# ajcm474/gapless-lossy-codec

Hardware: AMD Instinct MI355X
Metric: Msamples/s encoded (48 kHz stereo batch) at 1/2/4/8 GPUs; % HBM roofline (higher is better)
Workload: dtype f32; 1 GPU; BASELINE configs[1]: batch-encode 4096 frames x 1024 samples, 48 kHz stereo synthetic PCM (16-tone chord per channel) per GPU; frames_per_gpu=4096, channels=2, spinup_steps=500

## Files before the change

gapless-lossy-codec_amd/csrc/glc_api.hip:

```cpp
#include <hip/hip_runtime.h>

#include <algorithm>
#include <functional>
#include <cstdio>
#include <memory>
#include <mutex>
#include <new>
#include <string>
#include <cstdlib>
#include <vector>

#include "../../include/glc_debug.h"
#include "glc_args.hpp"
#include "glc_common.h"
#include "glc_kernels.h"
#include "glc_resources.hpp"
#include "glc_rounds.hpp"
#include "glc_stages.hpp"

namespace glc {

static std::mutex g_err_mu;
static std::string g_err;

// ... 48 lines not shown
  DevBuf rtb_stats;
  HostBuf rtb_stage;
  TableImage rtb_image;
  struct RtbClipInfo {
    uint64_t n_frames, stat_off;
    uint32_t stat_slots;
  };
  std::vector<RtbClipInfo> rtb_info;
  uint32_t rtb_info_ch = 0;
  DevBuf cd_status;
  uint64_t cd_status_n = 0;
  DevBuf sc_ws;
  DevBuf sc_stage;
  uint64_t sc_round = 0;
  HostBuf batch_stage;
  std::string err;
  glc::DecodeRows dec_rows{};
  uint64_t dec_uid = 0;
  uint32_t dec_delay = 0;
  uint64_t dec_orig_len = 0, dec_n_pairs = 0, dec_n_raw = 0;
  int d1_variant = 0;
  ScreenPolicy policy;
  HostBuf screen_stat;
  DevBuf edge_failed;
  DevBuf bound_tables;
  HostBuf probe_out;
  uint32_t dec_ch = 0;
  uint64_t dec_frames = 0, dec_next = 0;
  bool stream_open = false;
  int stream_elem = 0;
  DevBuf stream_out;
  int stream_buf = 0;
  uint64_t stream_frames = 0;
  bool stream_last = false;
  Stream own_stream;
  Stream stream;
  Stream copy_stream;
  Stream stream_b;
  Stream down_stream;
  Stream edge_stream;
  Stream probe_stream;
  Event ev_begin, ev_end;
  Event ev_fork, ev_join;
  std::vector<Event> ev_round;
  Event ev_dec[2];
  Event rtb_ev;
  Worker enc_up, enc_launch;
// ... 277 lines not shown
    const glc::SampleWindow need = glc::frame_sample_window(frame_begin, frame_end, plan.per_channel);
    if (need.hi > need.lo && (t0 > need.lo || t0 + t_count < need.hi))
      return fail(ctx, GLC_EINVAL, f + ": PCM shard does not cover the frame range (halo missing)");
  }
  return GLC_OK;
}

static hipError_t launch_quantize_decide(glc_ctx *ctx, const float *coef, const glc::PcmView &view,
                                         uint64_t frame_begin, uint64_t n_frames, uint8_t *records, hipStream_t st) {
  bool decided = false;
  hipError_t e = glc::launch_quantize(ctx->dev, coef, static_cast<uint32_t>(n_frames * view.ch), view.ch, view,
                                      frame_begin, records, st, &decided);
  if (e == hipSuccess && !decided)
    e = glc::launch_decide_raw(ctx->dev, view, frame_begin, static_cast<uint32_t>(n_frames), records, st);
  return e;
}

static hipError_t ensure_screen_shared(glc_ctx *ctx) {
  if (!ctx->screen_stat.p) {
    const hipError_t e = ctx->screen_stat.reserve(2 * 8 * sizeof(uint32_t));
    if (e != hipSuccess) return e;
    std::memset(ctx->screen_stat.p, 0, 2 * 8 * sizeof(uint32_t));
  }
  if (!ctx->edge_failed.p) {
    hipError_t e = ctx->edge_failed.reserve(2 * sizeof(uint64_t));
    if (e == hipSuccess) e = hipMemset(ctx->edge_failed.p, 0, 2 * sizeof(uint64_t));
    if (e == hipSuccess) e = hipStreamSynchronize(nullptr);
    if (e != hipSuccess) return e;
  }
  for (EncodeSlot &s : ctx->slot) {
    s.stat = static_cast<uint32_t *>(ctx->screen_stat.p) + 8 * s.index;
    s.failed_total = static_cast<unsigned long long *>(ctx->edge_failed.p) + s.index;
  }
  return hipSuccess;
}

static hipError_t reserve_slot(glc_ctx *ctx, EncodeSlot &slot, uint32_t ch, uint64_t frames, uint64_t chunk) {
  const uint64_t rows = std::min<uint64_t>(chunk, frames) * ch;
  hipError_t e = slot.coef.reserve(std::max<size_t>(rows, 1) * glc::kHop * sizeof(float));
  if (e == hipSuccess && ctx->policy.workspace_bytes(ch, frames, chunk)) e = ensure_screen_shared(ctx);
  if (e == hipSuccess) e = slot.reserve_screen(ctx->policy, ch, frames, chunk);
  return e;
}

static bool screen_takes(glc_ctx *ctx, uint32_t M, uint32_t ch) {
  ScreenPolicy &pol = ctx->policy;
  if (!pol.may(M, ch)) return false;
  bool pending = false;
  for (EncodeSlot &s : ctx->slot) {
    const volatile uint32_t *hs = s.stat;
    const uint32_t seq = hs[2], failed = hs[0], rows = hs[1];
    pol.observe(s.judged, seq, failed, rows);
    pending = pending || seq != s.seq;
  }
  return pol.admit(pending);
// ... 16 lines not shown
  if (alternate) {
    GLC_HIP(ctx, ctx->stream_b.ensure());
    GLC_HIP(ctx, ctx->ev_fork.ensure());
    GLC_HIP(ctx, ctx->ev_join.ensure());
    GLC_HIP(ctx, reserve_slot(ctx, ctx->slot[1], ch, frame_end - frame_begin, chunk));
    GLC_HIP(ctx, hipEventRecord(ctx->ev_fork, stream));
    GLC_HIP(ctx, hipStreamWaitEvent(ctx->stream_b, ctx->ev_fork, 0));
  }
  const glc_plan plan = glc::plan_encode(view.n_samples, static_cast<uint16_t>(ch));
  const glc::EdgeFrames ef = glc::edge_frames(plan.per_channel, plan.n_frames);
  uint64_t c_idx = 0;
  for (uint64_t f = frame_begin; f < frame_end; f += chunk, ++c_idx) {
    const uint64_t nf = std::min<uint64_t>(chunk, frame_end - f);
    const uint32_t M = static_cast<uint32_t>(nf * ch);
    const bool odd = alternate && (c_idx & 1);
    hipStream_t st = odd ? ctx->stream_b : stream;
    uint8_t *rp = recs + (f - frame_begin) * rec;
    EncodeSlot &slot = odd ? ctx->slot[1] : *r.slot;
    float *coef = d_coeffs ? d_coeffs + (f - frame_begin) * ch * glc::kHop : static_cast<float *>(slot.coef.p);
    if (!d_coeffs && screen_takes(ctx, M, ch)) {
      if (slot.screen_ws.cap < glc::encode_screen_bytes(M, pol.shape))
        return fail(ctx, GLC_EINVAL, "glc_encode_range_device: the screen's workspace was not reserved for this launch");
      bool decided = false;
      glc::ScreenLaunch sl{slot.screen_ws.p, slot.stat, 0, rp, st, pol.latency_repair(), pol.matrix_bound(M, ch), nullptr};
      if (slot.index == 0) pol.tap_rows = M, pol.tap_planes = sl.matrix_bound ? glc::MatrixBound::kGroups : pol.shape.n_planes;
      glc::EdgeLaunch edge{ef.a, ef.b, nullptr, nullptr, nullptr, nullptr, false, nullptr};
      const uint32_t n_edge = glc::edge_rows(ef.a, ef.b, f, M, ch).n;
      if ((flags & kEncodeEdge) && pol.edge_kind != 1 && n_edge >= 1 && n_edge <= glc::kEdgeRowsMax) {
        GLC_HIP(ctx, ctx->edge_stream.ensure());
        for (Event &ev : slot.ev_edge) GLC_HIP(ctx, ev.ensure());
        GLC_HIP(ctx, slot.edge_coef.reserve(static_cast<size_t>(glc::kEdgeRowsMax) * glc::kHop * sizeof(float)));
        edge.side = ctx->edge_stream;
        edge.ev_fork = slot.ev_edge[0], edge.ev_edge = slot.ev_edge[1];
        edge.coef = static_cast<float *>(slot.edge_coef.p);
        edge.capped = pol.edge_capped();
        edge.failed_total = slot.failed_total;
        ++pol.edge_launches;
        pol.edge_rows += n_edge;
        sl.edge = &edge;
      }
      sl.seq = ++slot.seq;
      GLC_HIP(ctx, glc::launch_encode_screened(ctx->dev, pol.shape, view, f, M, coef, sl, &decided));
      ++pol.repair_launches[sl.latency_repair ? 1 : 0];
      if (!decided) GLC_HIP(ctx, glc::launch_decide_raw(ctx->dev, view, f, static_cast<uint32_t>(nf), rp, st));
      pol.rows_screened += M;
      continue;
    }
    GLC_HIP(ctx, glc::launch_mdct_forward(ctx->dev, view, f, M, coef, st, pol.k1_variant, (flags & kEncodeBeside) != 0));
    GLC_HIP(ctx, launch_quantize_decide(ctx, coef, view, f, nf, rp, st));
  }
  if (alternate) {
    GLC_HIP(ctx, hipEventRecord(ctx->ev_join, ctx->stream_b));
    GLC_HIP(ctx, hipStreamWaitEvent(stream, ctx->ev_join, 0));
  }
  return GLC_OK;
}

int glc_encode_range_device(glc_ctx *ctx, const float *d_pcm, uint64_t t0, uint64_t t_count,
                            uint64_t n_samples, uint16_t channels, uint64_t frame_begin,
                            uint64_t frame_end, void *d_records, float *d_coeffs) {
  if (!ctx) return GLC_EINVAL;
  const EncodeRange r{{d_pcm, t0, t_count, n_samples, channels}, frame_begin, frame_end, d_records, d_coeffs, &ctx->slot[0]};
  return encode_range_on(ctx, ctx->stream, r, kEncodeAlternate | kEncodeEdge);
}

// ... 3276 lines not shown
  if (e == hipSuccess) e = hipMemcpy(d, p + 2048 + 4096, 4096, hipMemcpyDeviceToHost);
  GLC_HIP(ctx, e);
  return GLC_OK;
}

int glc_debug_encode_repair_stats(glc_ctx *ctx, uint64_t *launches_tiles, uint64_t *launches_latency) {
  if (!ctx || !launches_tiles || !launches_latency) return fail(ctx, GLC_EINVAL, "glc_debug_encode_repair_stats: null argument");
  *launches_tiles = ctx->policy.repair_launches[0];
  *launches_latency = ctx->policy.repair_launches[1];
  return GLC_OK;
}

int glc_debug_encode_screen_stats(glc_ctx *ctx, uint64_t *rows_screened, uint64_t *rows_repaired) {
  if (!ctx || !rows_screened || !rows_repaired) return fail(ctx, GLC_EINVAL, "glc_debug_encode_screen_stats: null argument");
  DeviceGuard guard(ctx->device);
  GLC_HIP(ctx, hipStreamSynchronize(ctx->stream));
  if (ctx->stream_b) GLC_HIP(ctx, hipStreamSynchronize(ctx->stream_b));
  *rows_screened = ctx->policy.rows_screened;
  *rows_repaired = 0;
  if (ctx->screen_stat.p) {
    const volatile uint64_t *hs = static_cast<const volatile uint64_t *>(ctx->screen_stat.p);
    *rows_repaired = hs[2] + hs[4 + 2];
  }
  if (ctx->edge_failed.p) {
    uint64_t e[2] = {0, 0};
    GLC_HIP(ctx, hipMemcpyAsync(e, ctx->edge_failed.p, sizeof e, hipMemcpyDeviceToHost, ctx->stream));
    GLC_HIP(ctx, hipStreamSynchronize(ctx->stream));
    *rows_repaired += e[0] + e[1];
  }
  return GLC_OK;
}

int glc_debug_encode_screen_layout(uint32_t ne, uint32_t rows, uint32_t *hybrid_pairs, uint32_t *planes,
                                   uint64_t *workspace_bytes) {
  if (!hybrid_pairs || !planes || !workspace_bytes) return GLC_EINVAL;
  const uint32_t edge = 64u * ne;
  glc::ScreenShape sh{};
  if (ne > 16 || !glc::encode_screen_shape(&edge, 1, &sh)) return GLC_EINVAL;
  *hybrid_pairs = sh.hp;
  *planes = sh.n_planes;
  *workspace_bytes = glc::encode_screen_bytes(rows, sh);
  return GLC_OK;
}

int glc_debug_clock_probe_begin(glc_ctx *ctx, uint32_t window_us) {
  if (!ctx || window_us == 0) return fail(ctx, GLC_EINVAL, "glc_debug_clock_probe_begin: bad argument");
  DeviceGuard guard(ctx->device);
  GLC_HIP(ctx, ctx->probe_stream.ensure());
  GLC_HIP(ctx, ctx->probe_out.reserve(64));
  std::memset(ctx->probe_out.p, 0, 16);
  GLC_HIP(ctx, glc::launch_clock_probe(static_cast<uint64_t>(window_us) * 100ull, static_cast<uint64_t *>(ctx->probe_out.p),
                                       ctx->probe_stream));
// ... 45 lines not shown
```

gapless-lossy-codec_amd/csrc/glc_kernels.h:

```cpp
#pragma once
#include <hip/hip_runtime.h>

#include <cstdint>

#include "glc_common.h"

namespace glc {

struct DeviceTables {
  const float *cos_t;
  const float *cos;
  const float *window;
  const float *indiv;
  const float *band_pf;
  const float *band_len;
  const uint16_t *band_of;
  const uint32_t *edges;
  uint32_t n_bands;
  float norm, cf, noise_floor;
  const uint16_t *cos_bf;
};

struct MatrixBound {
  static constexpr int kNe = 6;
// ... 22 lines not shown
};

hipError_t launch_mdct_forward(const DeviceTables &t, const PcmView &pcm, uint64_t frame_begin,
                               uint32_t M, float *coef, hipStream_t s, int variant = 0, bool beside = false);
hipError_t launch_quantize(const DeviceTables &t, const float *coef, uint32_t M, uint32_t ch, const PcmView &pcm,
                           uint64_t frame_begin, uint8_t *records, hipStream_t s, bool *decided);
struct ScreenShape {
  uint32_t l0, c0, ne;
  uint32_t hp;
  uint32_t n_planes;
};
bool encode_screen_shape(const uint32_t *edges, uint32_t n_bands, ScreenShape *sh);
bool mdct_forward_is_st16(uint32_t M, uint32_t ch, int variant);
bool mdct_forward_has_segment_loader(uint32_t ch);
uint64_t encode_screen_bytes(uint32_t M, const ScreenShape &sh);
struct EdgeLaunch {
  uint64_t a, b;
  hipStream_t side;
  hipEvent_t ev_fork, ev_edge;
  float *coef;
  bool capped;
  unsigned long long *failed_total;
};
struct ScreenLaunch {
  void *workspace;
  uint32_t *host_stat;
  uint32_t seq;
  uint8_t *records;
  hipStream_t s;
  bool latency_repair, matrix_bound;
  const EdgeLaunch *edge;
};
hipError_t launch_encode_screened(const DeviceTables &t, const ScreenShape &sh, const PcmView &pcm, uint64_t frame_begin,
                                  uint32_t M, float *coef, const ScreenLaunch &launch, bool *decided);

struct EdgeFrames {
  uint64_t a, b;
};
GLC_HD inline EdgeFrames edge_frames(uint64_t per_channel, uint64_t n_frames) {
  const uint64_t tail = kFrame - kHop / 2;
  uint64_t a = n_frames < 1 ? n_frames : 1;
  uint64_t b = per_channel >= tail ? (per_channel - tail) / kHop + 1 : 0;
  if (b > n_frames) b = n_frames;
  if (b < a) b = a;
  return {a, b};
}
struct EdgeRows {
  unsigned n_pre, suf0, n;
};
// ... 196 lines not shown
```

gapless-lossy-codec_amd/csrc/glc_kernels.hip:

```cpp
#include <algorithm>
#include <type_traits>

#include "glc_common.h"
#include "glc_kernels.h"
#include "glc_mdct_fwd.hpp"

#pragma clang fp contract(off)

namespace glc {

namespace {

template <int FALLBACK = 0, typename F>
auto by_channels(uint32_t ch, F &&f) {
  switch (ch) {
    case 1: return f(std::integral_constant<int, 1>{});
    case 2: return f(std::integral_constant<int, 2>{});
    case 4: return f(std::integral_constant<int, 4>{});
    case 8: return f(std::integral_constant<int, 8>{});
    default: return f(std::integral_constant<int, FALLBACK>{});
  }
}

constexpr int kHopI = 1024;
// ... 12 lines not shown
  return v.p[rel * v.ch + c];
}

__device__ __forceinline__ short sat_i16(float x) {
  if (x != x) return 0;
  x = fminf(fmaxf(x, -32768.0f), 32767.0f);
  return static_cast<short>(static_cast<int>(x));
}


constexpr int kQRows = 4;

constexpr float kScreenCErr = 2.45e-4f, kScreenSlack = 1.001f, kScreenTiny = 1e-33f;

struct ScreenArgs {
  const float *hf;
  unsigned *row_flag;
  unsigned *wave_fail;
  unsigned *host_stat;
  unsigned long long stride;
  unsigned c0, l0, n_planes, seq;
  unsigned long long edge_a, edge_b;
  unsigned long long *edge_total;
};

template <bool FUSED, int MODE>
__device__ __forceinline__ void quantize_body(const DeviceTables &tb, const float *__restrict__ coef, unsigned M,
                                              unsigned ch, unsigned long long rec_bytes, unsigned long long hdr_bytes,
                                              const PcmView &pcm, long long frame_begin,
                                              unsigned char *__restrict__ records, const ScreenArgs &sa) {
  __shared__ __attribute__((aligned(16))) float ssq[4][kQRows][kHopI];
  __shared__ float sbase[4][kQRows][64];
  const int w = threadIdx.x >> 6, lane = threadIdx.x & 63;
  unsigned blk = blockIdx.x;
  EdgeRows er{0u, M, 0u};
  if constexpr (MODE != 0) er = edge_rows(sa.edge_a, sa.edge_b, static_cast<unsigned long long>(frame_begin), M, ch);
  if constexpr (MODE == 3) {
    const unsigned g_pre = (er.n_pre + 15u) / 16u, g_suf = er.suf0 / 16u > g_pre ? er.suf0 / 16u : g_pre;
    if (blk >= g_pre) blk = g_suf + (blk - g_pre);
  }
  const unsigned m0 = (blk * 4 + w) * kQRows;
  unsigned on = 0;
  auto edge_row = [&](unsigned m) -> bool { return m < er.n_pre || m >= er.suf0; };
  if constexpr (MODE == 3) {
#pragma unroll
    for (int r = 0; r < kQRows; ++r)
      if (m0 + r < M && edge_row(m0 + r)) on |= 1u << r;
  }
  if constexpr (MODE == 2) {
    if (blk == 0 && w == 0) {
      const unsigned n_w = (M + 15) / 16 * 4;
      unsigned cnt = 0, ecnt = 0;
      unsigned long long etot = 0;
      if (er.n) etot = *sa.edge_total;
      for (unsigned i = lane; i < n_w; i += 64) cnt += sa.wave_fail[i];
      for (unsigned i = lane; i < er.n; i += 64) ecnt += sa.row_flag[i < er.n_pre ? i : er.suf0 + (i - er.n_pre)] == 2u;
#pragma unroll
      for (int off = 32; off > 0; off >>= 1) cnt += __shfl_xor(cnt, off), ecnt += __shfl_xor(ecnt, off);
      if (lane == 0) {
        volatile unsigned *hs = sa.host_stat;
        volatile unsigned long long *tot = reinterpret_cast<volatile unsigned long long *>(sa.host_stat + 4);
        *tot = *tot + cnt;
        if (er.n) *sa.edge_total = etot + ecnt;
        hs[0] = cnt;
        hs[1] = M;
        hs[2] = sa.seq;
      }
    }
    const unsigned fr = blk * 16 + lane;
    const bool flagged = lane < 16 && fr < M && sa.row_flag[fr] == 1u;
    const unsigned blk_on = static_cast<unsigned>(__ballot(flagged));
    if (blk_on == 0u) return;
    on = (blk_on >> (4 * w)) & 0xFu;
  }
  auto row_on = [&](int r) -> bool {
    if constexpr (MODE == 0) return m0 + r < M;
    else return (on >> r) & 1u;
  };

  float4 indiv4[4];
  unsigned short bo[4][4];
#pragma unroll
  for (int j = 0; j < 4; ++j) {
    const int k0 = (lane + 64 * j) * 4;
    indiv4[j] = *reinterpret_cast<const float4 *>(tb.indiv + k0);
    const ushort4 b4 = *reinterpret_cast<const ushort4 *>(tb.band_of + k0);
    bo[j][0] = b4.x; bo[j][1] = b4.y; bo[j][2] = b4.z; bo[j][3] = b4.w;
  }

  float4 c4[kQRows][4];
  float scale[kQRows];
// ... 56 lines not shown
      const bool pass = __ballot(hit) == 0ull && bound <= nfl && bound < __builtin_inff();
      if (!pass) fail |= 1u << r;
    }
    unsigned valid = 0;
#pragma unroll
    for (int r = 0; r < kQRows; ++r)
      if (m0 + r < M) valid |= 1u << r;
    fail &= valid;
    if (FUSED) {
      unsigned ff = 0;
#pragma unroll
      for (int r = 0; r < kQRows; ++r)
#pragma unroll
        for (int q = 0; q < kQRows; ++q)
          if (static_cast<unsigned>(q) / ch == static_cast<unsigned>(r) / ch && ((fail >> q) & 1u)) ff |= 1u << r;
      fail = ff & valid;
    }
    unsigned edge = 0;
#pragma unroll
    for (int r = 0; r < kQRows; ++r)
      if (((valid >> r) & 1u) && edge_row(m0 + r)) edge |= 1u << r;
    on = valid & ~fail & ~edge;
    if (lane < kQRows && m0 + lane < M) sa.row_flag[m0 + lane] = ((fail >> lane) & 1u) << ((edge >> lane) & 1u);
    if (lane == 0) sa.wave_fail[blk * 4 + w] = __builtin_popcount(fail & ~edge);
  }
  __syncthreads();

  {
    const int r = lane >> 4;
    if (row_on(r)) {
      const float *sq = ssq[w][r];
      for (unsigned b = lane & 15; b < tb.n_bands; b += 16) {
        if constexpr (MODE == 1) {
          if (b == tb.n_bands - 1) {
            sbase[w][r][b] = 0.0f;
            continue;
          }
        }
        const unsigned lo = tb.edges[b], hi = tb.edges[b + 1];
        float ss = 0.0f;
        unsigned i = lo;
        for (; i < hi && (i & 3u); ++i) ss = add_rn(ss, sq[i]);
#define GLC_ADD4(V) ss = add_rn(ss, V.x); ss = add_rn(ss, V.y); ss = add_rn(ss, V.z); ss = add_rn(ss, V.w)
        if (i + 16 <= hi) {
          const float4 *q4 = reinterpret_cast<const float4 *>(sq);
          float4 a0 = q4[i >> 2], a1 = q4[(i >> 2) + 1], a2 = q4[(i >> 2) + 2], a3 = q4[(i >> 2) + 3];
          while (i + 32 <= hi) {
            const float4 b0 = q4[(i >> 2) + 4], b1 = q4[(i >> 2) + 5], b2 = q4[(i >> 2) + 6], b3 = q4[(i >> 2) + 7];
            GLC_ADD4(a0); GLC_ADD4(a1); GLC_ADD4(a2); GLC_ADD4(a3);
// ... 1768 lines not shown
}

hipError_t launch_debug_mfma_bf16(const uint16_t *a, const uint16_t *b, const float *c, float *d, hipStream_t s) {
  hipLaunchKernelGGL(k_debug_mfma_bf16, dim3(1), dim3(64), 0, s, a, b, c, d);
  return hipGetLastError();
}

bool encode_matrix_bound_built(const DeviceTables &t, const ScreenShape &sh, uint32_t ch) {
  return t.cos_bf && sh.ne == static_cast<uint32_t>(MatrixBound::kNe) && (ch == 1 || ch == 2 || ch == 4 || ch == 8);
}

namespace {
inline uint64_t screen_stride(uint32_t M) { return (static_cast<uint64_t>(M) + 255ull) / 256ull * 256ull; }
}

uint64_t encode_screen_bytes(uint32_t M, const ScreenShape &sh) {
  return ((sh.n_planes + 1ull) * screen_stride(M) + screen_stride(M) + screen_stride(M) / 4) * 4ull;
}

hipError_t launch_encode_screened(const DeviceTables &t, const ScreenShape &sh, const PcmView &pcm, uint64_t frame_begin,
                                  uint32_t M, float *coef, const ScreenLaunch &launch, bool *decided) {
  void *const workspace = launch.workspace;
  uint32_t *const host_stat = launch.host_stat;
  const uint32_t seq = launch.seq;
  uint8_t *const records = launch.records;
  const hipStream_t s = launch.s;
  const bool latency_repair = launch.latency_repair, matrix_bound = launch.matrix_bound;
  const EdgeLaunch *const edge = launch.edge;
  *decided = pcm.ch == 1 || pcm.ch == 2 || pcm.ch == 4;
  if (M == 0) return hipSuccess;
  const unsigned long long edge_a = edge ? edge->a : 0ull, edge_b = edge ? edge->b : kNoEdge;
  const EdgeRows er = edge_rows(edge_a, edge_b, frame_begin, M, pcm.ch);
  if (edge && (er.n == 0 || er.n > kEdgeRowsMax || !edge->side || edge->side == s || !edge->coef || !edge->failed_total))
    return hipErrorInvalidValue;
  const uint64_t stride = screen_stride(M);
  float *hf = static_cast<float *>(workspace);
  unsigned *row_flag = reinterpret_cast<unsigned *>(hf + (sh.n_planes + 1ull) * stride);
  unsigned *wave_fail = row_flag + stride;
  static_assert(MatrixBound::kGroups <= 8, "the matrix form's planes fit in those of any FMA form (8 at the least)");
  if (matrix_bound && !encode_matrix_bound_built(t, sh, pcm.ch)) return hipErrorInvalidValue;
  const unsigned n_planes = matrix_bound ? static_cast<unsigned>(MatrixBound::kGroups) : sh.n_planes;
  hipError_t e;
  if (edge && (e = hipEventRecord(edge->ev_fork, s)) != hipSuccess) return e;
  if (matrix_bound)
    e = by_channels<8>(pcm.ch, [&](auto CH) {
      return k1::launch_mx_st<decltype(CH)::value>(t, pcm, frame_begin, M, coef, hf, stride, s);
    });
  else
    e = by_channels(pcm.ch, [&](auto CH) {
      return k1::launch_mix_st<decltype(CH)::value>(t, pcm, frame_begin, M, coef, sh.ne, sh.hp, hf, stride, s);
    });
  if (e != hipSuccess) return e;
  const ScreenArgs sa{hf, row_flag, wave_fail, host_stat, stride, sh.c0, sh.l0, n_planes, seq, edge_a, edge_b,
                      edge ? edge->failed_total : nullptr};
  const unsigned long long hdr = record_header_bytes(pcm.ch), rec = record_bytes(pcm.ch);
  const dim3 grid((M + 4 * kQRows - 1) / (4 * kQRows));
  const long long fb = static_cast<long long>(frame_begin);
  bool forked = false;
  auto leave = [&](hipError_t err) -> hipError_t {
    if (!forked) return err;
    hipError_t j = hipEventRecord(edge->ev_edge, edge->side);
    if (j == hipSuccess) j = hipStreamWaitEvent(s, edge->ev_edge, 0);
    return err != hipSuccess ? err : j;
  };
  if (edge) {
    if ((e = hipStreamWaitEvent(edge->side, edge->ev_fork, 0)) != hipSuccess) return e;
    forked = true;
    e = edge->capped ? k1::launch_edge_rows<GLC_SMALL_ROWS_R, true>(t, pcm, frame_begin, M, edge->coef, er, 0u, edge->side)
                     : k1::launch_edge_rows<GLC_SMALL_ROWS_R, false>(t, pcm, frame_begin, M, edge->coef, er, 0u, edge->side);
    if (e != hipSuccess) return leave(e);
    const unsigned g_pre = (er.n_pre + 15u) / 16u, g_suf = std::max(er.suf0 / 16u, g_pre), g_end = (M + 15u) / 16u;
    const dim3 egrid(g_pre + (er.suf0 < M && g_suf < g_end ? g_end - g_suf : 0u));
    if (*decided)
      hipLaunchKernelGGL((k_quantize_screen<true, 3>), egrid, dim3(256), 0, edge->side, t, edge->coef, M, pcm.ch, rec, hdr, pcm, fb, records, sa);
    else
      hipLaunchKernelGGL((k_quantize_screen<false, 3>), egrid, dim3(256), 0, edge->side, t, edge->coef, M, pcm.ch, rec, hdr, pcm, fb, records, sa);
    if ((e = hipGetLastError()) != hipSuccess) return leave(e);
  }
  if (*decided)
    hipLaunchKernelGGL((k_quantize_screen<true, 1>), grid, dim3(256), 0, s, t, coef, M, pcm.ch, rec, hdr, pcm, fb, records, sa);
  else
    hipLaunchKernelGGL((k_quantize_screen<false, 1>), grid, dim3(256), 0, s, t, coef, M, pcm.ch, rec, hdr, pcm, fb, records, sa);
  if ((e = hipGetLastError()) != hipSuccess) return leave(e);
  e = latency_repair ? k1::launch_small_rows<GLC_SMALL_ROWS_R>(t, pcm, frame_begin, M, coef, row_flag, wave_fail, sh.c0, s)
                     : k1::launch_small_cols<2>(t, pcm, frame_begin, M, coef, row_flag, sh.c0, s);
  if (e != hipSuccess) return leave(e);
  if (*decided)
    hipLaunchKernelGGL((k_quantize_screen<true, 2>), grid, dim3(256), 0, s, t, coef, M, pcm.ch, rec, hdr, pcm, fb, records, sa);
  else
    hipLaunchKernelGGL((k_quantize_screen<false, 2>), grid, dim3(256), 0, s, t, coef, M, pcm.ch, rec, hdr, pcm, fb, records, sa);
  return leave(hipGetLastError());
}

hipError_t launch_quantize(const DeviceTables &t, const float *coef, uint32_t M, uint32_t ch, const PcmView &pcm,
                           uint64_t frame_begin, uint8_t *records, hipStream_t s, bool *decided) {
  *decided = ch == 1 || ch == 2 || ch == 4;
  if (M == 0) return hipSuccess;
  const unsigned long long hdr = record_header_bytes(ch), rec = record_bytes(ch);
  const dim3 grid((M + 4 * kQRows - 1) / (4 * kQRows));
  if (*decided)
    hipLaunchKernelGGL(k_quantize<true>, grid, dim3(256), 0, s, t, coef, M, ch, rec, hdr, pcm,
                       static_cast<long long>(frame_begin), records);
  else
    hipLaunchKernelGGL(k_quantize<false>, grid, dim3(256), 0, s, t, coef, M, ch, rec, hdr, pcm,
                       static_cast<long long>(frame_begin), records);
  return hipGetLastError();
}
// ... 520 lines not shown
```

gapless-lossy-codec_amd/csrc/glc_mdct_fwd.hpp:

```cpp
#pragma once
#include <hip/hip_runtime.h>

#include <type_traits>

#include "glc_kernels.h"

namespace glc {
namespace k1 {

constexpr int kHopI = 1024;
constexpr int kFrameI = 2048;

__device__ __forceinline__ float mul_rn(float a, float b) { return __fmul_rn(a, b); }
__device__ __forceinline__ float add_rn(float a, float b) { return __fadd_rn(a, b); }

typedef float f32x2 __attribute__((ext_vector_type(2)));
typedef float f32x4 __attribute__((ext_vector_type(4)));

template <typename Row, typename Ch>
__device__ __forceinline__ long long pcm_frame_first(const PcmView &pcm, long long frame_begin, Row row, Ch ch) {
  const long long f = frame_begin + row / ch;
  return (f * kHopI - kHopI / 2 - static_cast<long long>(pcm.t0)) * ch;
}
template <typename Ch>
// ... 1766 lines not shown
}

__device__ __forceinline__ void rows_mac4(f32x2 &acc, f32x4 xa, f32x4 xb, f32x4 t) {
  const f32x2 x0 = __builtin_shufflevector(xa, xa, 0, 1), x1 = __builtin_shufflevector(xa, xa, 2, 3);
  const f32x2 x2 = __builtin_shufflevector(xb, xb, 0, 1), x3 = __builtin_shufflevector(xb, xb, 2, 3);
  const f32x2 t01 = __builtin_shufflevector(t, t, 0, 1), t23 = __builtin_shufflevector(t, t, 2, 3);
  f32x2 p0, p1, p2, p3;
  asm volatile(
      "v_pk_mul_f32 %1, %5, %9 op_sel_hi:[1,0]\n\t"
      "v_pk_mul_f32 %2, %6, %9 op_sel:[0,1]\n\t"
      "v_pk_add_f32 %0, %0, %1\n\t"
      "v_pk_mul_f32 %3, %7, %10 op_sel_hi:[1,0]\n\t"
      "v_pk_add_f32 %0, %0, %2\n\t"
      "v_pk_mul_f32 %4, %8, %10 op_sel:[0,1]\n\t"
      "v_pk_add_f32 %0, %0, %3\n\t"
      "v_pk_add_f32 %0, %0, %4"
      : "+v"(acc), "=&v"(p0), "=&v"(p1), "=&v"(p2), "=&v"(p3)
      : "v"(x0), "v"(x1), "v"(x2), "v"(x3), "v"(t01), "v"(t23));
}

template <int R, bool FROM_ARGS, int NB = 8>
__device__ __forceinline__ void small_rows_body(const DeviceTables &tb, const PcmView &pcm, long long frame_begin, unsigned M,
                                                float *__restrict__ coef, const unsigned *__restrict__ row_flag,
                                                const unsigned *__restrict__ wave_fail, unsigned col0, const EdgeRows er) {
  static_assert(R == 2 || R == 4, "rows of a group: whole packed pairs");
  constexpr int NP = R / 2;
  constexpr unsigned kNone = 0xFFFFFFFFu;
  __shared__ __attribute__((aligned(16))) float xs[NP * kFrameI * 2];
  __shared__ unsigned s_row[R], s_total;
  const unsigned lane = threadIdx.x;

  const unsigned n_w = (M + 15u) / 16u * 4u;
  const unsigned per = ((n_w + 63u) / 64u + 3u) & ~3u;
  const unsigned w0 = lane * per;
  const uint4 *wf4 = reinterpret_cast<const uint4 *>(wave_fail);
  auto counts = [&](unsigned w) -> uint4 {
    const bool in = w < per && w0 + w < n_w;
    const uint4 c = wf4[in ? (w0 + w) >> 2 : 0u];
    return in ? c : uint4{0u, 0u, 0u, 0u};
  };
  unsigned cnt = 0, base = 0, n_fail = er.n;
  if constexpr (!FROM_ARGS) {
    for (unsigned w = 0; w < per; w += 32) {
      uint4 c[8];
#pragma unroll
      for (int k = 0; k < 8; ++k) c[k] = counts(w + 4 * k);
#pragma unroll
      for (int k = 0; k < 8; ++k) cnt += c[k].x + c[k].y + c[k].z + c[k].w;
    }
    unsigned incl = cnt;
#pragma unroll
    for (int off = 1; off < 64; off <<= 1) {
      const unsigned v = __shfl_up(incl, off);
// ... 121 lines not shown
        else rows_issue_x<NP>(X[0], xa_next, 0);
#pragma unroll
        for (int j = 0; j < 4; ++j)
#pragma unroll
          for (int p = 0; p < NP; ++p) rows_mac4(acc[p], X[b & 1].v[p][2 * j], X[b & 1].v[p][2 * j + 1], T[b][j]);
        rows_wait_x<NP>(X[(b + 1) & 1]);
      }
      tp = tp_next;
      xa = xa_next;
    }
    asm volatile("s_waitcnt vmcnt(0)" ::: "memory");

#pragma unroll
    for (int q = 0; q < R; ++q)
      if (m[q] != kNone)
        coef[static_cast<size_t>(FROM_ARGS ? g * R + q : m[q]) * kHopI + col] = mul_rn(q & 1 ? acc[q >> 1].y : acc[q >> 1].x, tb.norm);
    if constexpr (FROM_ARGS) break;
  }
}

template <int R>
__global__ __launch_bounds__(64) void k_mdct_fwd_small_rows(DeviceTables tb, PcmView pcm, long long frame_begin, unsigned M,
                                                             float *__restrict__ coef, const unsigned *__restrict__ row_flag,
                                                             const unsigned *__restrict__ wave_fail, unsigned col0) {
  small_rows_body<R, false>(tb, pcm, frame_begin, M, coef, row_flag, wave_fail, col0, EdgeRows{0u, M, 0u});
}

template <int R>
__global__ __launch_bounds__(64) void k_mdct_edge_rows(DeviceTables tb, PcmView pcm, long long frame_begin, unsigned M,
                                                        float *__restrict__ coef, unsigned col0, EdgeRows er) {
  small_rows_body<R, true, 8>(tb, pcm, frame_begin, M, coef, nullptr, nullptr, col0, er);
}

constexpr int kEdgeCapVgprs = 192;
template <int R>
__global__ __launch_bounds__(64) __attribute__((amdgpu_num_vgpr(kEdgeCapVgprs))) void k_mdct_edge_rows_capped(
    DeviceTables tb, PcmView pcm, long long frame_begin, unsigned M, float *__restrict__ coef, unsigned col0, EdgeRows er) {
  small_rows_body<R, true, 4>(tb, pcm, frame_begin, M, coef, nullptr, nullptr, col0, er);
}

template <int R>
inline hipError_t launch_small_rows(const DeviceTables &t, const PcmView &pcm, uint64_t frame_begin, uint32_t M, float *coef,
                                    const unsigned *row_flag, const unsigned *wave_fail, uint32_t col0, hipStream_t s) {
  if (M == 0 || col0 >= static_cast<uint32_t>(kHopI)) return hipSuccess;
  if (col0 % 64u || !row_flag || !wave_fail) return hipErrorInvalidValue;
  hipLaunchKernelGGL((k_mdct_fwd_small_rows<R>), dim3(kRowsGrid), dim3(64), 0, s, t, pcm, static_cast<long long>(frame_begin), M,
                     coef, row_flag, wave_fail, col0);
  return hipGetLastError();
}

template <int R, bool CAPPED>
inline hipError_t launch_edge_rows(const DeviceTables &t, const PcmView &pcm, uint64_t frame_begin, uint32_t M, float *coef,
                                   const EdgeRows &er, uint32_t col0, hipStream_t s) {
  if (M == 0 || er.n == 0 || col0 >= static_cast<uint32_t>(kHopI)) return hipSuccess;
  if (col0 % 64u || er.n_pre > er.suf0 || er.suf0 > M || er.n != er.n_pre + (M - er.suf0)) return hipErrorInvalidValue;
  const unsigned n_items = (er.n + R - 1) / R * ((static_cast<unsigned>(kHopI) - col0) / kRowsSlab);
  if (CAPPED)
    hipLaunchKernelGGL((k_mdct_edge_rows_capped<R>), dim3(n_items), dim3(64), 0, s, t, pcm, static_cast<long long>(frame_begin), M,
                       coef, col0, er);
  else
    hipLaunchKernelGGL((k_mdct_edge_rows<R>), dim3(n_items), dim3(64), 0, s, t, pcm, static_cast<long long>(frame_begin), M, coef,
                       col0, er);
  return hipGetLastError();
}

template <int BM, int BN, int BK, int TM, int TN, int UNROLL, int MINW>
inline hipError_t launch(const DeviceTables &t, const PcmView &pcm, uint64_t frame_begin, uint32_t M,
                         float *coef, hipStream_t s) {
  using C = Cfg<BM, BN, BK, TM, TN, UNROLL, MINW>;
  if (M == 0) return hipSuccess;
// ... 9 lines not shown
```

gapless-lossy-codec_amd/csrc/glc_resources.hpp:

```cpp
#pragma once
#include <hip/hip_runtime.h>

#include <algorithm>
#include <atomic>
#include <cstdint>
#include <utility>

#include "glc_kernels.h"

namespace glc {

enum LiveKind { kLiveDevBuf = 0, kLivePinnedBuf, kLiveStream, kLiveEvent, kLiveKinds };
inline std::atomic<uint64_t> g_live[kLiveKinds];
inline void live_add(LiveKind k) { g_live[k].fetch_add(1, std::memory_order_relaxed); }
inline void live_sub(LiveKind k) { g_live[k].fetch_sub(1, std::memory_order_relaxed); }

}

struct DevBuf {
  void *p = nullptr;
  size_t cap = 0;
  DevBuf() = default;
  DevBuf(DevBuf &&o) noexcept : p(std::exchange(o.p, nullptr)), cap(std::exchange(o.cap, 0)) {}
  DevBuf &operator=(DevBuf &&o) noexcept {
// ... 135 lines not shown

  bool matrix_bound(uint32_t M, uint32_t ch) const {
    if (bound_kind == 1 || !glc::encode_matrix_bound_built(*dev, shape, ch)) return false;
    return bound_kind == 2 || M >= 3584u;
  }

  uint64_t workspace_bytes(uint32_t ch, uint64_t frames, uint64_t chunk) const {
    const uint32_t m_full = static_cast<uint32_t>(std::min(chunk, frames) * ch);
    const uint32_t m_last = frames > chunk ? static_cast<uint32_t>(frames % chunk * ch) : 0u;
    uint64_t need = 0;
    if (may(m_full, ch)) need = glc::encode_screen_bytes(m_full, shape);
    if (m_last && may(m_last, ch)) need = std::max(need, glc::encode_screen_bytes(m_last, shape));
    return need;
  }
};

struct EncodeSlot {
  int index = 0;
  DevBuf coef;
  DevBuf screen_ws;
  uint32_t *stat = nullptr;
  uint32_t seq = 0, judged = 0;
  DevBuf edge_coef;
  unsigned long long *failed_total = nullptr;
  Event ev_edge[2];

  hipError_t reserve_screen(const ScreenPolicy &policy, uint32_t ch, uint64_t frames, uint64_t chunk) {
    const uint64_t need = policy.workspace_bytes(ch, frames, chunk);
    return need ? screen_ws.reserve(need) : hipSuccess;
  }
};
```

include/glc_debug.h:

```cpp
#ifndef GLC_DEBUG_H
#define GLC_DEBUG_H

#include "glc.h"

#ifdef __cplusplus
extern "C" {
#endif

int glc_debug_set_imdct_variant(glc_ctx *ctx, int variant);

int glc_debug_set_mdct_variant(glc_ctx *ctx, int variant);

int glc_debug_set_encode_screen(glc_ctx *ctx, int mode);
int glc_debug_encode_screen_stats(glc_ctx *ctx, uint64_t *rows_screened, uint64_t *rows_repaired);
int glc_debug_encode_screen_layout(uint32_t ne, uint32_t rows, uint32_t *hybrid_pairs, uint32_t *planes,
                                   uint64_t *workspace_bytes);

int glc_debug_set_encode_repair(glc_ctx *ctx, int kind);
int glc_debug_encode_repair_stats(glc_ctx *ctx, uint64_t *launches_tiles, uint64_t *launches_latency);

int glc_debug_set_encode_edge(glc_ctx *ctx, int kind);
int glc_debug_encode_edge_stats(glc_ctx *ctx, uint64_t *launches, uint64_t *rows);

int glc_debug_set_encode_bound(glc_ctx *ctx, int kind);
int glc_debug_encode_bound_tap(glc_ctx *ctx, uint32_t rows, float *h, float *a);
int glc_debug_mfma_bf16(glc_ctx *ctx, const uint16_t *a, const uint16_t *b, const float *c, float *d);
int glc_debug_encode_matrix_bound(uint32_t *ne, uint32_t *pieces, uint32_t *products, uint32_t *k_block, uint32_t *seg_blocks,
                                  uint32_t *planes, double *kappa, double *split_eps, double *budget);

int glc_debug_quantize_device(glc_ctx *ctx, const float *d_coeffs, const float *d_pcm, uint64_t t0, uint64_t t_count,
                              uint64_t n_samples, uint16_t channels, uint64_t frame_begin, uint64_t frame_end,
                              void *d_records);

int glc_debug_overlap_add_device(glc_ctx *ctx, const float *d_blocks, int64_t blk_frame0, uint64_t n_block_frames,
                                 uint64_t n_frames, uint16_t channels, uint64_t hop_begin, uint64_t hop_end, float *d_out,
                                 uint64_t cap);

// ... 35 lines not shown
```

Before: 26930 Msamples/s.

## Track screen failures in a device word and skip repair work when none fail

The screening quantize pass now accumulates per-block failure counts into a double-buffered device word indexed by launch sequence. Later stages read that word: the MODE 2 finalize kernel no longer reduces the whole wave_fail array, and both it and the small-rows repair kernel return early when the count is zero. This removes repair and reduction work on clean batches, at the cost of one atomic per block and extra state that must be reset, which is handled by a dirty flag with a memset after a failed launch.

```diff
diff --git a/gapless-lossy-codec_amd/csrc/glc_api.hip b/gapless-lossy-codec_amd/csrc/glc_api.hip
--- a/gapless-lossy-codec_amd/csrc/glc_api.hip
+++ b/gapless-lossy-codec_amd/csrc/glc_api.hip
@@ -94,7 +94,7 @@
   int d1_variant = 0;
   ScreenPolicy policy;
   HostBuf screen_stat;
-  DevBuf edge_failed;
+  DevBuf screen_words;
   DevBuf bound_tables;
   HostBuf probe_out;
   uint32_t dec_ch = 0;
@@ -418,15 +418,15 @@
     if (e != hipSuccess) return e;
     std::memset(ctx->screen_stat.p, 0, 2 * 8 * sizeof(uint32_t));
   }
-  if (!ctx->edge_failed.p) {
-    hipError_t e = ctx->edge_failed.reserve(2 * sizeof(uint64_t));
-    if (e == hipSuccess) e = hipMemset(ctx->edge_failed.p, 0, 2 * sizeof(uint64_t));
+  if (!ctx->screen_words.p) {
+    hipError_t e = ctx->screen_words.reserve(2 * sizeof(glc::ScreenWords));
+    if (e == hipSuccess) e = hipMemset(ctx->screen_words.p, 0, 2 * sizeof(glc::ScreenWords));
     if (e == hipSuccess) e = hipStreamSynchronize(nullptr);
     if (e != hipSuccess) return e;
   }
   for (EncodeSlot &s : ctx->slot) {
     s.stat = static_cast<uint32_t *>(ctx->screen_stat.p) + 8 * s.index;
-    s.failed_total = static_cast<unsigned long long *>(ctx->edge_failed.p) + s.index;
+    s.words = static_cast<glc::ScreenWords *>(ctx->screen_words.p) + s.index;
   }
   return hipSuccess;
 }
@@ -489,7 +489,7 @@
       if (slot.screen_ws.cap < glc::encode_screen_bytes(M, pol.shape))
         return fail(ctx, GLC_EINVAL, "glc_encode_range_device: the screen's workspace was not reserved for this launch");
       bool decided = false;
-      glc::ScreenLaunch sl{slot.screen_ws.p, slot.stat, 0, rp, st, pol.latency_repair(), pol.matrix_bound(M, ch), nullptr};
+      glc::ScreenLaunch sl{slot.screen_ws.p, slot.stat, slot.words, 0, rp, st, pol.latency_repair(), pol.matrix_bound(M, ch), nullptr};
       if (slot.index == 0) pol.tap_rows = M, pol.tap_planes = sl.matrix_bound ? glc::MatrixBound::kGroups : pol.shape.n_planes;
       glc::EdgeLaunch edge{ef.a, ef.b, nullptr, nullptr, nullptr, nullptr, false, nullptr};
       const uint32_t n_edge = glc::edge_rows(ef.a, ef.b, f, M, ch).n;
@@ -501,13 +501,19 @@
         edge.ev_fork = slot.ev_edge[0], edge.ev_edge = slot.ev_edge[1];
         edge.coef = static_cast<float *>(slot.edge_coef.p);
         edge.capped = pol.edge_capped();
-        edge.failed_total = slot.failed_total;
+        edge.failed_total = &slot.words->edge_total;
         ++pol.edge_launches;
         pol.edge_rows += n_edge;
         sl.edge = &edge;
       }
+      if (slot.words_dirty) {
+        GLC_HIP(ctx, hipMemsetAsync(slot.words->fail_word, 0, sizeof slot.words->fail_word, st));
+        slot.words_dirty = false;
+      }
       sl.seq = ++slot.seq;
-      GLC_HIP(ctx, glc::launch_encode_screened(ctx->dev, pol.shape, view, f, M, coef, sl, &decided));
+      const hipError_t se = glc::launch_encode_screened(ctx->dev, pol.shape, view, f, M, coef, sl, &decided);
+      slot.words_dirty = se != hipSuccess;
+      GLC_HIP(ctx, se);
       ++pol.repair_launches[sl.latency_repair ? 1 : 0];
       if (!decided) GLC_HIP(ctx, glc::launch_decide_raw(ctx->dev, view, f, static_cast<uint32_t>(nf), rp, st));
       pol.rows_screened += M;
@@ -3830,12 +3836,26 @@
     const volatile uint64_t *hs = static_cast<const volatile uint64_t *>(ctx->screen_stat.p);
     *rows_repaired = hs[2] + hs[4 + 2];
   }
-  if (ctx->edge_failed.p) {
-    uint64_t e[2] = {0, 0};
-    GLC_HIP(ctx, hipMemcpyAsync(e, ctx->edge_failed.p, sizeof e, hipMemcpyDeviceToHost, ctx->stream));
+  if (ctx->screen_words.p) {
+    glc::ScreenWords w[2] = {};
+    GLC_HIP(ctx, hipMemcpyAsync(w, ctx->screen_words.p, sizeof w, hipMemcpyDeviceToHost, ctx->stream));
     GLC_HIP(ctx, hipStreamSynchronize(ctx->stream));
-    *rows_repaired += e[0] + e[1];
-  }
+    *rows_repaired += w[0].edge_total + w[1].edge_total;
+  }
+  return GLC_OK;
+}
+
+int glc_debug_encode_screen_words(glc_ctx *ctx, int slot, uint32_t words[2], uint32_t *seq, uint64_t *fail_total) {
+  if (!ctx || slot < 0 || slot > 1 || !words || !seq || !fail_total || !ctx->screen_words.p)
+    return fail(ctx, GLC_EINVAL, "glc_debug_encode_screen_words: bad argument, or no screened launch on this context yet");
+  DeviceGuard guard(ctx->device);
+  GLC_HIP(ctx, hipStreamSynchronize(ctx->stream));
+  if (ctx->stream_b) GLC_HIP(ctx, hipStreamSynchronize(ctx->stream_b));
+  glc::ScreenWords w{};
+  GLC_HIP(ctx, hipMemcpy(&w, static_cast<const glc::ScreenWords *>(ctx->screen_words.p) + slot, sizeof w, hipMemcpyDeviceToHost));
+  words[0] = w.fail_word[0], words[1] = w.fail_word[1];
+  *seq = ctx->slot[slot].seq;
+  *fail_total = w.fail_total;
   return GLC_OK;
 }
 
diff --git a/gapless-lossy-codec_amd/csrc/glc_kernels.h b/gapless-lossy-codec_amd/csrc/glc_kernels.h
--- a/gapless-lossy-codec_amd/csrc/glc_kernels.h
+++ b/gapless-lossy-codec_amd/csrc/glc_kernels.h
@@ -68,9 +68,16 @@
   bool capped;
   unsigned long long *failed_total;
 };
+struct ScreenWords {
+  unsigned long long edge_total;
+  unsigned long long fail_total;
+  unsigned fail_word[2];
+  unsigned pad[2];
+};
 struct ScreenLaunch {
   void *workspace;
   uint32_t *host_stat;
+  ScreenWords *words;
   uint32_t seq;
   uint8_t *records;
   hipStream_t s;
diff --git a/gapless-lossy-codec_amd/csrc/glc_kernels.hip b/gapless-lossy-codec_amd/csrc/glc_kernels.hip
--- a/gapless-lossy-codec_amd/csrc/glc_kernels.hip
+++ b/gapless-lossy-codec_amd/csrc/glc_kernels.hip
@@ -58,6 +58,8 @@
   unsigned c0, l0, n_planes, seq;
   unsigned long long edge_a, edge_b;
   unsigned long long *edge_total;
+  unsigned *fail_word;
+  unsigned long long *fail_total;
 };
 
 template <bool FUSED, int MODE>
@@ -67,6 +69,7 @@
                                               unsigned char *__restrict__ records, const ScreenArgs &sa) {
   __shared__ __attribute__((aligned(16))) float ssq[4][kQRows][kHopI];
   __shared__ float sbase[4][kQRows][64];
+  __shared__ unsigned s_fail[4];
   const int w = threadIdx.x >> 6, lane = threadIdx.x & 63;
   unsigned blk = blockIdx.x;
   EdgeRows er{0u, M, 0u};
@@ -84,25 +87,28 @@
       if (m0 + r < M && edge_row(m0 + r)) on |= 1u << r;
   }
   if constexpr (MODE == 2) {
+    const unsigned cnt = sa.fail_word[sa.seq & 1u];
     if (blk == 0 && w == 0) {
-      const unsigned n_w = (M + 15) / 16 * 4;
-      unsigned cnt = 0, ecnt = 0;
-      unsigned long long etot = 0;
-      if (er.n) etot = *sa.edge_total;
-      for (unsigned i = lane; i < n_w; i += 64) cnt += sa.wave_fail[i];
-      for (unsigned i = lane; i < er.n; i += 64) ecnt += sa.row_flag[i < er.n_pre ? i : er.suf0 + (i - er.n_pre)] == 2u;
-#pragma unroll
-      for (int off = 32; off > 0; off >>= 1) cnt += __shfl_xor(cnt, off), ecnt += __shfl_xor(ecnt, off);
+      if (er.n) {
+        unsigned ecnt = 0;
+        const unsigned long long etot = *sa.edge_total;
+        for (unsigned i = lane; i < er.n; i += 64) ecnt += sa.row_flag[i < er.n_pre ? i : er.suf0 + (i - er.n_pre)] == 2u;
+#pragma unroll
+        for (int off = 32; off > 0; off >>= 1) ecnt += __shfl_xor(ecnt, off);
+        if (lane == 0) *sa.edge_total = etot + ecnt;
+      }
       if (lane == 0) {
+        sa.fail_word[(sa.seq & 1u) ^ 1u] = 0u;
+        const unsigned long long total = *sa.fail_total + cnt;
+        *sa.fail_total = total;
         volatile unsigned *hs = sa.host_stat;
-        volatile unsigned long long *tot = reinterpret_cast<volatile unsigned long long *>(sa.host_stat + 4);
-        *tot = *tot + cnt;
-        if (er.n) *sa.edge_total = etot + ecnt;
+        *reinterpret_cast<volatile unsigned long long *>(sa.host_stat + 4) = total;
         hs[0] = cnt;
         hs[1] = M;
         hs[2] = sa.seq;
       }
     }
+    if (cnt == 0u) return;
     const unsigned fr = blk * 16 + lane;
     const bool flagged = lane < 16 && fr < M && sa.row_flag[fr] == 1u;
     const unsigned blk_on = static_cast<unsigned>(__ballot(flagged));
@@ -205,9 +211,19 @@
       if (((valid >> r) & 1u) && edge_row(m0 + r)) edge |= 1u << r;
     on = valid & ~fail & ~edge;
     if (lane < kQRows && m0 + lane < M) sa.row_flag[m0 + lane] = ((fail >> lane) & 1u) << ((edge >> lane) & 1u);
-    if (lane == 0) sa.wave_fail[blk * 4 + w] = __builtin_popcount(fail & ~edge);
+    if (lane == 0) {
+      const unsigned n1 = __builtin_popcount(fail & ~edge);
+      sa.wave_fail[blk * 4 + w] = n1;
+      s_fail[w] = n1;
+    }
   }
   __syncthreads();
+  if constexpr (MODE == 1) {
+    if (threadIdx.x == 0) {
+      const unsigned n1 = s_fail[0] + s_fail[1] + s_fail[2] + s_fail[3];
+      if (n1) atomicAdd(sa.fail_word + (sa.seq & 1u), n1);
+    }
+  }
 
   {
     const int r = lane >> 4;
@@ -2022,6 +2038,7 @@
                                   uint32_t M, float *coef, const ScreenLaunch &launch, bool *decided) {
   void *const workspace = launch.workspace;
   uint32_t *const host_stat = launch.host_stat;
+  ScreenWords *const words = launch.words;
   const uint32_t seq = launch.seq;
   uint8_t *const records = launch.records;
   const hipStream_t s = launch.s;
@@ -2029,6 +2046,7 @@
   const EdgeLaunch *const edge = launch.edge;
   *decided = pcm.ch == 1 || pcm.ch == 2 || pcm.ch == 4;
   if (M == 0) return hipSuccess;
+  if (!words) return hipErrorInvalidValue;
   const unsigned long long edge_a = edge ? edge->a : 0ull, edge_b = edge ? edge->b : kNoEdge;
   const EdgeRows er = edge_rows(edge_a, edge_b, frame_begin, M, pcm.ch);
   if (edge && (er.n == 0 || er.n > kEdgeRowsMax || !edge->side || edge->side == s || !edge->coef || !edge->failed_total))
@@ -2052,7 +2070,7 @@
     });
   if (e != hipSuccess) return e;
   const ScreenArgs sa{hf, row_flag, wave_fail, host_stat, stride, sh.c0, sh.l0, n_planes, seq, edge_a, edge_b,
-                      edge ? edge->failed_total : nullptr};
+                      edge ? edge->failed_total : nullptr, words->fail_word, &words->fail_total};
   const unsigned long long hdr = record_header_bytes(pcm.ch), rec = record_bytes(pcm.ch);
   const dim3 grid((M + 4 * kQRows - 1) / (4 * kQRows));
   const long long fb = static_cast<long long>(frame_begin);
@@ -2082,7 +2100,8 @@
   else
     hipLaunchKernelGGL((k_quantize_screen<false, 1>), grid, dim3(256), 0, s, t, coef, M, pcm.ch, rec, hdr, pcm, fb, records, sa);
   if ((e = hipGetLastError()) != hipSuccess) return leave(e);
-  e = latency_repair ? k1::launch_small_rows<GLC_SMALL_ROWS_R>(t, pcm, frame_begin, M, coef, row_flag, wave_fail, sh.c0, s)
+  const unsigned *const fail_word = words->fail_word + (seq & 1u);
+  e = latency_repair ? k1::launch_small_rows<GLC_SMALL_ROWS_R>(t, pcm, frame_begin, M, coef, row_flag, wave_fail, fail_word, sh.c0, s)
                      : k1::launch_small_cols<2>(t, pcm, frame_begin, M, coef, row_flag, sh.c0, s);
   if (e != hipSuccess) return leave(e);
   if (*decided)
diff --git a/gapless-lossy-codec_amd/csrc/glc_mdct_fwd.hpp b/gapless-lossy-codec_amd/csrc/glc_mdct_fwd.hpp
--- a/gapless-lossy-codec_amd/csrc/glc_mdct_fwd.hpp
+++ b/gapless-lossy-codec_amd/csrc/glc_mdct_fwd.hpp
@@ -1812,13 +1812,17 @@
 template <int R, bool FROM_ARGS, int NB = 8>
 __device__ __forceinline__ void small_rows_body(const DeviceTables &tb, const PcmView &pcm, long long frame_begin, unsigned M,
                                                 float *__restrict__ coef, const unsigned *__restrict__ row_flag,
-                                                const unsigned *__restrict__ wave_fail, unsigned col0, const EdgeRows er) {
+                                                const unsigned *__restrict__ wave_fail, const unsigned *__restrict__ fail_word,
+                                                unsigned col0, const EdgeRows er) {
   static_assert(R == 2 || R == 4, "rows of a group: whole packed pairs");
   constexpr int NP = R / 2;
   constexpr unsigned kNone = 0xFFFFFFFFu;
   __shared__ __attribute__((aligned(16))) float xs[NP * kFrameI * 2];
   __shared__ unsigned s_row[R], s_total;
   const unsigned lane = threadIdx.x;
+  if constexpr (!FROM_ARGS) {
+    if (*fail_word == 0u) return;
+  }
 
   const unsigned n_w = (M + 15u) / 16u * 4u;
   const unsigned per = ((n_w + 63u) / 64u + 3u) & ~3u;
@@ -1986,30 +1990,32 @@
 template <int R>
 __global__ __launch_bounds__(64) void k_mdct_fwd_small_rows(DeviceTables tb, PcmView pcm, long long frame_begin, unsigned M,
                                                              float *__restrict__ coef, const unsigned *__restrict__ row_flag,
-                                                             const unsigned *__restrict__ wave_fail, unsigned col0) {
-  small_rows_body<R, false>(tb, pcm, frame_begin, M, coef, row_flag, wave_fail, col0, EdgeRows{0u, M, 0u});
+                                                             const unsigned *__restrict__ wave_fail,
+                                                             const unsigned *__restrict__ fail_word, unsigned col0) {
+  small_rows_body<R, false>(tb, pcm, frame_begin, M, coef, row_flag, wave_fail, fail_word, col0, EdgeRows{0u, M, 0u});
 }
 
 template <int R>
 __global__ __launch_bounds__(64) void k_mdct_edge_rows(DeviceTables tb, PcmView pcm, long long frame_begin, unsigned M,
                                                         float *__restrict__ coef, unsigned col0, EdgeRows er) {
-  small_rows_body<R, true, 8>(tb, pcm, frame_begin, M, coef, nullptr, nullptr, col0, er);
+  small_rows_body<R, true, 8>(tb, pcm, frame_begin, M, coef, nullptr, nullptr, nullptr, col0, er);
 }
 
 constexpr int kEdgeCapVgprs = 192;
 template <int R>
 __global__ __launch_bounds__(64) __attribute__((amdgpu_num_vgpr(kEdgeCapVgprs))) void k_mdct_edge_rows_capped(
     DeviceTables tb, PcmView pcm, long long frame_begin, unsigned M, float *__restrict__ coef, unsigned col0, EdgeRows er) {
-  small_rows_body<R, true, 4>(tb, pcm, frame_begin, M, coef, nullptr, nullptr, col0, er);
+  small_rows_body<R, true, 4>(tb, pcm, frame_begin, M, coef, nullptr, nullptr, nullptr, col0, er);
 }
 
 template <int R>
 inline hipError_t launch_small_rows(const DeviceTables &t, const PcmView &pcm, uint64_t frame_begin, uint32_t M, float *coef,
-                                    const unsigned *row_flag, const unsigned *wave_fail, uint32_t col0, hipStream_t s) {
+                                    const unsigned *row_flag, const unsigned *wave_fail, const unsigned *fail_word, uint32_t col0,
+                                    hipStream_t s) {
   if (M == 0 || col0 >= static_cast<uint32_t>(kHopI)) return hipSuccess;
-  if (col0 % 64u || !row_flag || !wave_fail) return hipErrorInvalidValue;
+  if (col0 % 64u || !row_flag || !wave_fail || !fail_word) return hipErrorInvalidValue;
   hipLaunchKernelGGL((k_mdct_fwd_small_rows<R>), dim3(kRowsGrid), dim3(64), 0, s, t, pcm, static_cast<long long>(frame_begin), M,
-                     coef, row_flag, wave_fail, col0);
+                     coef, row_flag, wave_fail, fail_word, col0);
   return hipGetLastError();
 }
 
diff --git a/gapless-lossy-codec_amd/csrc/glc_resources.hpp b/gapless-lossy-codec_amd/csrc/glc_resources.hpp
--- a/gapless-lossy-codec_amd/csrc/glc_resources.hpp
+++ b/gapless-lossy-codec_amd/csrc/glc_resources.hpp
@@ -181,7 +181,8 @@
   uint32_t *stat = nullptr;
   uint32_t seq = 0, judged = 0;
   DevBuf edge_coef;
-  unsigned long long *failed_total = nullptr;
+  glc::ScreenWords *words = nullptr;
+  bool words_dirty = false;
   Event ev_edge[2];
 
   hipError_t reserve_screen(const ScreenPolicy &policy, uint32_t ch, uint64_t frames, uint64_t chunk) {
diff --git a/include/glc_debug.h b/include/glc_debug.h
--- a/include/glc_debug.h
+++ b/include/glc_debug.h
@@ -13,6 +13,7 @@
 
 int glc_debug_set_encode_screen(glc_ctx *ctx, int mode);
 int glc_debug_encode_screen_stats(glc_ctx *ctx, uint64_t *rows_screened, uint64_t *rows_repaired);
+int glc_debug_encode_screen_words(glc_ctx *ctx, int slot, uint32_t words[2], uint32_t *seq, uint64_t *fail_total);
 int glc_debug_encode_screen_layout(uint32_t ne, uint32_t rows, uint32_t *hybrid_pairs, uint32_t *planes,
                                    uint64_t *workspace_bytes);
 
```

Result: no change. 26840 Msamples/s (-0.4%).
